# RobotControlLab/nimblephysics

Measured on AMD Instinct MI355X. Metric: differentiable timesteps/sec (fwd+bwd), 1024-env Atlas w/ contact, higher is better.
Workload: dtype f64; 1 GPU; Atlas 33-DoF (atlas_v3_box_colliders) + ground, foot contact; worlds_per_gpu=1024, dofs=33, global_batch=1024, parallelism=independent worlds x1, launcher=single process

## Files before the change

### nimblephysics_amd/csrc/capi.cpp

```cpp
#include <hip/hip_runtime.h>

#include <cmath>
#include <cstdlib>
#include <cstdio>
#include <cstring>
#include <string>
#include <vector>

#include "model.h"
#include "pool_sizes.h"

static thread_local std::string g_err;

static int fail(int code, const std::string& msg) {
  g_err = msg;
  return code;
}

#define HIP_TRY(expr)                                                        \
  do {                                                                       \
    hipError_t _e = (expr);                                                  \
    if (_e != hipSuccess) return fail(NIMBLE_ERR_HIP, std::string(#expr) + ": " + hipGetErrorString(_e)); \
  } while (0)

// ... 106 lines not shown
  m.ns = d->num_shapes;
  m.dt = d->dt;
  for (int i = 0; i < 3; i++) m.g[i] = d->gravity[i];
  m.clipDepth = d->contact_clipping_depth;
  m.fallbackCfm = d->fallback_cfm;
  m.penCorr = d->penetration_correction;
  m.parallelPosVel = d->parallel_pos_vel;
  int dofCount = 0;
  for (int b = 0; b < m.nb; b++) {
    int p = d->parent[b];
    if (p >= b) { delete w; return fail(NIMBLE_ERR_INVALID, "bodies must be in topological order"); }
    m.parent[b] = p;
    m.jtype[b] = d->joint_type[b];
    m.dof0[b] = d->dof_offset[b];
    m.ndof[b] = jointDofs(m.jtype[b]);
    if (m.ndof[b] < 0) { delete w; return fail(NIMBLE_ERR_INVALID, "unknown joint type"); }
    m.depth[b] = p >= 0 ? m.depth[p] + 1 : 0;
    if (m.depth[b] > m.maxDepth) m.maxDepth = m.depth[b];
    m.anc[b] = (p >= 0 ? m.anc[p] : 0ull) | (1ull << b);
    m.skel[b] = d->skeleton[b];
    std::memcpy(m.Tpj[b], d->T_parent_joint + 12 * b, 12 * sizeof(double));
    std::memcpy(m.Tcj[b], d->T_child_joint + 12 * b, 12 * sizeof(double));
    isoInverse(m.Tcj[b], m.TcjInv[b]);
    for (int i = 0; i < 3; i++) m.axis[b][i] = d->axis[3 * b + i];
    m.mass[b] = d->mass[b];
    for (int i = 0; i < 3; i++) m.com[b][i] = d->com[3 * b + i];
    const double* mo = d->moment + 6 * b;
    double I[9] = {mo[0], mo[3], mo[4], mo[3], mo[1], mo[5], mo[4], mo[5], mo[2]};
    std::memcpy(m.Ic[b], I, sizeof(I));
    m.friction[b] = d->friction[b];
    m.restitution[b] = d->restitution[b];
    for (int k = 0; k < m.ndof[b]; k++) m.dofBody[m.dof0[b] + k] = b;
    dofCount += m.ndof[b];
    if (m.jtype[b] == NIMBLE_JOINT_FREE || m.jtype[b] == NIMBLE_JOINT_BALL) {
      if (m.numFree >= 8) { delete w; return fail(NIMBLE_ERR_UNSUPPORTED, "more than 8 free / ball joints"); }
      m.freeBody[m.numFree++] = b;
    }
  }
  if (dofCount != m.n) { delete w; return fail(NIMBLE_ERR_INVALID, "dof count mismatch"); }
  {
    int k = 0;
    for (int lev = 0; lev <= m.maxDepth; lev++) {
      m.levelStart[lev] = k;
      for (int b = 0; b < m.nb; b++)
        if (m.depth[b] == lev) m.levelBodies[k++] = b;
    }
    m.levelStart[m.maxDepth + 1] = k;
    k = 0;
    for (int p = 0; p < m.nb; p++) {
      m.childStart[p] = k;
      for (int b = 0; b < m.nb; b++)
        if (m.parent[b] == p) m.childList[k++] = b;
    }
    m.childStart[m.nb] = k;
    k = 0;
    for (int lev = m.maxDepth; lev >= 1; lev--)
      for (int b = 0; b < m.nb; b++)
        if (m.depth[b] == lev && m.parent[b] >= 0) { m.accEdge[k][0] = m.parent[b]; m.accEdge[k][1] = b; k++; }
    m.numAcc = k;
  }
  for (int b = 0; b < m.nb; b++) {
    bool hasDof = false;
    for (int a = b; a >= 0; a = m.parent[a]) if (m.ndof[a] > 0) { hasDof = true; break; }
    m.reactive[b] = (d->skeleton_mobile[b] && hasDof) ? 1 : 0;
  }
  for (int i = 0; i < m.n; i++) {
    m.damping[i] = d->damping[i]; m.spring[i] = d->spring[i]; m.rest[i] = d->rest_position[i];
    m.posLo[i] = d->pos_lower[i]; m.posHi[i] = d->pos_upper[i];
    m.velLo[i] = d->vel_lower[i]; m.velHi[i] = d->vel_upper[i];
    m.forceLo[i] = d->force_lower[i]; m.forceHi[i] = d->force_upper[i];
  }
  for (int sIdx = 0; sIdx < m.ns; sIdx++) {
    m.shapeBody[sIdx] = d->shape_body[sIdx];
    m.shapeType[sIdx] = d->shape_type[sIdx];
    for (int i = 0; i < 3; i++) m.shapeSize[sIdx][i] = d->shape_size[3 * sIdx + i];
    std::memcpy(m.shapeT[sIdx], d->shape_T + 12 * sIdx, 12 * sizeof(double));
  }
  m.helperPrio = 0;
  if (const char* e = getenv("NIMBLE_AMD_HELPER_PRIO")) m.helperPrio = atoi(e) & 3;
  m.postSplit = 1;
  if (const char* e = getenv("NIMBLE_AMD_POST_SPLIT")) m.postSplit = atoi(e) != 0;
  m.pinvMfma = 1;
  if (const char* e = getenv("NIMBLE_AMD_PINV_MFMA")) m.pinvMfma = atoi(e) != 0 ? 1 : 0;
  m.guardSites = 0;
  m.guardStride = 1;
  m.guardOffset = 0;
  if (const char* e = getenv("NIMBLE_AMD_GUARD_TEST")) {
    int sites = 0, stride = 1, offset = 0;
    if (sscanf(e, "%d:%d:%d", &sites, &stride, &offset) >= 1 && stride > 0 && offset >= 0 && offset < stride) {
      m.guardSites = sites;
      m.guardStride = stride;
      m.guardOffset = offset;
    }
  }
  m.numPairs = 0;
  m.pairChunk = 0;
  for (int i = 0; i < m.ns; i++)
    for (int j = i + 1; j < m.ns; j++) {
      int bi = m.shapeBody[i], bj = m.shapeBody[j];
      if (bi == bj) continue;
      int si = m.skel[bi], sj = m.skel[bj];
      if (!d->skeleton_mobile[bi] && !d->skeleton_mobile[bj]) continue;
      if (si == sj) continue;
      m.pairA[m.numPairs] = i;
      m.pairB[m.numPairs] = j;
      m.numPairs++;
    }
  m.pairChunk = m.numPairs < CT_PAIR_CHUNK_HOST ? m.numPairs : CT_PAIR_CHUNK_HOST;
  {
    std::vector<double> mv;
    m.hasMesh = 0;
    for (int sIdx = 0; sIdx < m.ns; sIdx++) {
      m.meshFirst[sIdx] = 0; m.meshCount[sIdx] = 0; m.meshRadius[sIdx] = 0.0;
      if (m.shapeType[sIdx] != NIMBLE_SHAPE_MESH) continue;
      if (d->mesh_vertices == nullptr || d->shape_mesh_count == nullptr || d->shape_mesh_count[sIdx] <= 0) {
        delete w;
        return fail(NIMBLE_ERR_INVALID, "mesh shape without vertices");
      }
      const int f = d->shape_mesh_first[sIdx], c = d->shape_mesh_count[sIdx];
      if (f < 0 || f + c > d->num_mesh_vertices) { delete w; return fail(NIMBLE_ERR_INVALID, "mesh vertex range"); }
      m.meshFirst[sIdx] = (int)(mv.size() / 3);
      double r2 = 0.0;
      for (int k = 0; k < c; k++) {
        const double* v = d->mesh_vertices + 3 * (size_t)(f + k);
        double q = 0.0;
        for (int i = 0; i < 3; i++) q += (v[i] * m.shapeSize[sIdx][i]) * (v[i] * m.shapeSize[sIdx][i]);
        if (q > r2) r2 = q;
        if (d->mesh_vertex_candidate != nullptr && d->mesh_vertex_candidate[f + k] == 0) continue;
        mv.insert(mv.end(), v, v + 3);
      }
      m.meshCount[sIdx] = (int)(mv.size() / 3) - m.meshFirst[sIdx];
      m.meshRadius[sIdx] = std::sqrt(r2);
      if (m.meshCount[sIdx] <= 0) {
        delete w;
        return fail(NIMBLE_ERR_INVALID, "mesh_vertex_candidate filters out every vertex of a mesh shape");
      }
    }
    if (!mv.empty()) {
      hipError_t e = hipMalloc(&w->meshDev, mv.size() * sizeof(double));
      if (e == hipSuccess) e = hipMemcpy(w->meshDev, mv.data(), mv.size() * sizeof(double), hipMemcpyHostToDevice);
      if (e != hipSuccess) {
        if (w->meshDev) (void)hipFree(w->meshDev);
        delete w;
        return fail(NIMBLE_ERR_HIP, std::string("mesh upload: ") + hipGetErrorString(e));
      }
    }
    m.meshVerts = w->meshDev;
    for (int p = 0; p < m.numPairs; p++)
      if (m.shapeType[m.pairA[p]] == NIMBLE_SHAPE_MESH || m.shapeType[m.pairB[p]] == NIMBLE_SHAPE_MESH) m.hasMesh = 1;
    if (m.hasMesh) m.pairChunk = m.numPairs > 0 ? 1 : 0;
  }
  int maxContacts = m.hasMesh ? NIMBLE_MAX_CONTACTS : 8 * m.numPairs;
  if (maxContacts > NIMBLE_MAX_CONTACTS) maxContacts = NIMBLE_MAX_CONTACTS;
  m.maxContacts = maxContacts;
  const int mcap = 3 * maxContacts < NIMBLE_MAX_SOLVED_LCP ? 3 * maxContacts : NIMBLE_MAX_SOLVED_LCP;
  if (const char* e = getenv("NIMBLE_AMD_DEFER_ROWS")) {
    const int d = atoi(e);
    if (d >= 0 && d < w->deferRows) w->deferRows = d;
  }
  int fwdRows = ldsPoolRows(m, mcap);
  for (;;) {
    w->fwd = makeLayout(m, false, fwdRows);
    if (w->fwd.total * 8 <= 160 * 1024) break;
    if (fwdRows == 0) {
      if (w->meshDev) (void)hipFree(w->meshDev);
      delete w;
// ... 251 lines not shown
```

### nimblephysics_amd/csrc/contact.cuh

```cuda
#pragma once
#include "model.h"
#include "spatial.cuh"
#include "pool_sizes.h"
#include "capsule.cuh"
#include "mesh.cuh"

#define CT_FACE_VERTEX 1
#define CT_VERTEX_FACE 2
#define CT_EDGE_EDGE 3
#include "stamp.cuh"

#define CM_CLAMPING (-1)
#define CM_NOT_CLAMPING (-2)


__device__ int deviceBoxBox(const double* p1, const double* R1, const double* A, const double* p2,
                            const double* R2, const double* B, double clipDepth, int b1, int b2, double* out) {
#pragma clang fp contract(off)
  const double fudge = 1.05;
  double p[3] = {p2[0] - p1[0], p2[1] - p1[1], p2[2] - p1[2]};
  double pp[3];
  for (int i = 0; i < 3; i++) pp[i] = R1[i] * p[0] + R1[3 + i] * p[1] + R1[6 + i] * p[2];
  double Rm[9], Qm[9];
  for (int i = 0; i < 3; i++)
// ... 2612 lines not shown
    }
  }
  const double tn = sqrt(dot3(t, t));
  for (int i = 0; i < 3; i++) t[i] /= tn;
  double gc[3];
  cross3(cr, g, gc);
  for (int i = 0; i < 3; i++) gc[i] /= tn;
  double gt[3];
  if (fabs(tn - 1.0) > 1e-6) {
    const double dd = dot3(gc, t);
    for (int i = 0; i < 3; i++) gt[i] = gc[i] - dd * t[i];
  } else {
    for (int i = 0; i < 3; i++) gt[i] = gc[i];
  }
  double a[3], b[3];
  cross3(g, t, a);
  cross3(nrm, gt, b);
  for (int i = 0; i < 3; i++) { T0[i] = gt[i]; T1[i] = a[i] + b[i]; }
}

template <int R = 1>
__device__ int contactBackwardPrep(const ModelDev& md, double* s, const Layout& L, int lane, const double* sn,
                                   BwdPool& P, int m, int nc, double* ct, int fcRow) {
  const int n = md.n;
  const double dt = md.dt;
  const double* rows = sn + SN_ROWS;
  const double* Ac = sn + snAc(n);
  const double* AcubE = sn + snAcubE(n);
  const double* PT = sn + snPT(n);
  const double* Q = sn + snQ(n);
  const double* Lm = s + L.M;
  const double* dinv = s + L.dinv;
  const int imp = uni((int)sn[SN_IMP]);
#ifdef NIMBLE_STAGE_TIMING
  double* g_stamp = (double*)sn + snStamps(n);
#endif
  STAMP(30);
  (void)ct;
  for (int j = lane; j < m; j += WAVE)
    if ((int)rows[j * SN_ROWREC + RR_MAP] == CM_CLAMPING) P.rowOf[(int)rows[j * SN_ROWREC + RR_CIDX]] = j;
  WSYNC();
  for (int c = lane; c < nc; c += WAVE) {
    const int r = P.rowOf[c];
    P.fc[c] = sn[SN_FC + c];
    P.bc[c] = rows[r * SN_ROWREC + RR_B];
    P.bounce[c] = rows[r * SN_ROWREC + RR_BOUNCE];
  }
  WSYNC();
  for (int c = lane; c < nc; c += WAVE) {
    double xx = 0;
#pragma unroll 8
    for (int r = 0; r < nc; r++) xx += PT[r * nc + c] * P.bc[r];
    P.xq[c] = xx;
  }
  WSYNC();
  for (int c = lane; c < nc; c += WAVE) {
    double qx = 0, ze = 0;
    if (imp)
#pragma unroll 8
      for (int k = 0; k < nc; k++) {
        qx += Q[c * nc + k] * P.xq[k];
        ze += PT[c * nc + k] * P.xq[k];
      }
    P.r1[c] = imp ? P.bc[c] - qx : 0.0;
    P.zeta[c] = imp ? ze : 0.0;
  }
  WSYNC();
  STAMP(31);
  {
    double X[5] = {0, 0, 0, 0, 0};
    if (lane < n) {
      X[0] = s[L.gv + lane];
      double a1 = 0, a2 = 0, a3 = 0, a4 = 0;
#pragma unroll 8
      for (int c = 0; c < nc; c++) {
        const double ae = AcubE[lane * nc + c], ac = Ac[lane * nc + c];
        a1 += ae * P.fc[c];
        a2 += ae * P.xq[c];
        a3 += ac * P.r1[c];
        a4 += ac * P.zeta[c];
      }
      X[1] = a1; X[2] = a2; X[3] = a3; X[4] = a4;
    }
    cholSolveReg<5>(Lm, dinv, X, n, lane);
    if (lane < n) {
      double* nv = P.NV + lane * NV_COLS;
      const double d = X[1] / dt;
      nv[NV_W] = X[0];
      nv[NV_DELTA] = d;
      nv[NV_SIGMA] = X[2];
      nv[NV_MA1] = X[3];
      nv[NV_MA2] = X[4];
      s[L.w + lane] = X[0];
      s[L.x + lane] = sn[snYf(n) + lane] + d;
    }
  }
  WSYNC();
  for (int c = lane; c < nc; c += WAVE) {
    double acc = 0;
#pragma unroll 8
    for (int i = 0; i < n; i++) acc += AcubE[i * nc + c] * s[L.w + i];
    P.u[c] = fcRow >= 0 ? (c == fcRow ? 1.0 : 0.0) : acc;
  }
  WSYNC();
  for (int c = lane; c < nc; c += WAVE) {
    double l = 0;
#pragma unroll 8
    for (int r = 0; r < nc; r++) l += PT[c * nc + r] * P.u[r];
    P.lam[c] = l;
    P.beta[c] = P.bounce[c] * l;
  }
  WSYNC();
  for (int c = lane; c < nc; c += WAVE) {
    double qtl = 0, rh = 0;
    if (imp)
#pragma unroll 8
      for (int k = 0; k < nc; k++) {
        qtl += Q[k * nc + c] * P.lam[k];
        rh += PT[k * nc + c] * P.lam[k];
      }
    P.piv[c] = imp ? P.u[c] - qtl : 0.0;
    P.rho[c] = imp ? rh : 0.0;
  }
  WSYNC();
  STAMP(35);
  {
    double X[4] = {0, 0, 0, 0};
    double mu = 0;
    if (lane < n) {
      double a0 = 0, a1 = 0, a2 = 0, a3 = 0;
#pragma unroll 8
      for (int c = 0; c < nc; c++) {
        const double ae = AcubE[lane * nc + c], ac = Ac[lane * nc + c];
        a0 += ac * P.beta[c];
        a1 += ac * P.lam[c];
        a2 += ae * P.rho[c];
        a3 += ae * P.piv[c];
      }
      X[0] = a0; X[1] = a1; X[2] = a2; X[3] = a3;
      mu = a0;
    }
    cholSolveReg<4>(Lm, dinv, X, n, lane);
    if (lane < n) {
      double* nv = P.NV + lane * NV_COLS;
      nv[NV_MU] = mu;
      nv[NV_NU] = X[0];
      nv[NV_KAPPA] = X[1];
      nv[NV_MARHO] = X[2];
      nv[NV_MAPI] = X[3];
      const double w2 = nv[NV_W] - X[0];
      nv[NV_W2] = w2;
      s[L.w + lane] = w2;
    }
  }
  WSYNC();
  STAMP(37);
  int rMap[R], rC[R];
  double rE[R];
#pragma unroll
  for (int q = 0; q < R; q++) {
    const int j = rowAt(q, lane);
    rMap[q] = CM_NOT_CLAMPING;
    rC[q] = 0;
    rE[q] = 0.0;
    if (j < m) {
      const double* rr = rows + j * SN_ROWREC;
      rMap[q] = (int)rr[RR_MAP];
      if (rMap[q] == CM_CLAMPING) rC[q] = (int)rr[RR_CIDX];
      else if (rMap[q] >= 0) { rC[q] = (int)rows[rMap[q] * SN_ROWREC + RR_CIDX]; rE[q] = rr[RR_EVAL]; }
    }
  }
  {
    const int i = lane;
    const bool live = i < n;
    const double* nv = P.NV + (live ? i : 0) * NV_COLS;
    const double w = nv[NV_W], sg = nv[NV_SIGMA], ka = nv[NV_KAPPA], ma1 = nv[NV_MA1], mar = nv[NV_MARHO];
    const double ma2 = nv[NV_MA2], map = nv[NV_MAPI], vf = sn[SN_VF + (live ? i : 0)];
    for (int j = 0; j < m; j++) {
      const int mp = rdliR(rMap, j);
      const int c = rdliR(rC, j);
      const double e = rdlR(rE, j);
      double g = 0.0;
      if (mp == CM_CLAMPING) {
        g = P.fc[c] * w - P.beta[c] * vf - P.lam[c] * sg - P.xq[c] * ka;
        if (imp) g += P.rho[c] * ma1 + P.r1[c] * mar + P.piv[c] * ma2 + P.zeta[c] * map;
      } else if (mp >= 0) {
        double inner = P.fc[c] * w - P.xq[c] * ka;
        if (imp) inner += P.rho[c] * ma1 + P.piv[c] * ma2;
        g = e * inner;
      }
      if (live) P.gRows[j * n + i] = g;
    }
  }
  WSYNC();
  {
    auto bodyOf = [&](int t) {
      if (t >= 2 * m) return -1;
      const double* rec = sn + SN_CONTACTS + (int)rows[(t >> 1) * SN_ROWREC + RR_CONTACT] * CREC;
      return (int)rec[8 + (t & 1)];
    };
    unsigned long long anAll = 0ull;
    for (int t = lane; t < 2 * m; t += WAVE) {
      const int body = bodyOf(t);
      if (body >= 0) anAll |= md.anc[body];
    }
    unsigned lo = (unsigned)anAll, hi = (unsigned)(anAll >> 32);
    for (int o = 32; o >= 1; o >>= 1) {
      lo |= __shfl_xor(lo, o);
      hi |= __shfl_xor(hi, o);
    }
    const unsigned long long all = ((unsigned long long)uni((int)hi) << 32) | (unsigned)uni((int)lo);
    const unsigned long long dmAll = ancestorDofMask(md, all, lane);
    for (int t0 = 0; t0 < 2 * m; t0 += WAVE) {
      const int t = t0 + lane;
      const int body = bodyOf(t);
      const unsigned long long an = body >= 0 ? md.anc[body] : 0ull;
      unsigned long long dm = dmAll;
      double T[6] = {0, 0, 0, 0, 0, 0};
      const double* g = P.gRows + (t < 2 * m ? (t >> 1) : 0) * n;
      while (dm) {
        const int r = __ffsll((long long)dm) - 1;
        dm &= dm - 1ull;
        const double gr = ((an >> md.dofBody[r]) & 1ull) ? g[r] : 0.0;
        for (int i = 0; i < 6; i++) T[i] = fma(s[L.Sw + 6 * r + i], gr, T[i]);
// ... 511 lines not shown
      {
        unsigned long long dm = ancestorDofMask(md, md.anc[c], lane);
        if (lane < nb) {
          double pb[6] = {0, 0, 0, 0, 0, 0};
          const unsigned long long an = md.anc[lane];
          while (dm) {
            const int r = __ffsll((long long)dm) - 1;
            dm &= dm - 1ull;
            const double w = ((an >> md.dofBody[r]) & 1ull) ? 1.0 : 0.0;
#pragma unroll
            for (int i = 0; i < 6; i++) pb[i] = fma(w, omega[6 * r + i], pb[i]);
          }
          for (int i = 0; i < 6; i++) Pc[lane * 6 + i] = pb[i];
        }
      }
      WSYNC();
      if (k < n && ((md.anc[c] >> bk) & 1ull)) {
        double y[6];
        for (int i = 0; i < 6; i++) y[i] = Pc[c * 6 + i] - (lam >= 0 ? Pc[lam * 6 + i] : 0.0);
        acc += dot6(Z, y);
        const double zw = sqrt(Z[0] * Z[0] + Z[1] * Z[1] + Z[2] * Z[2]);
        if (zw > 1e-6) acc += Z[0] * UV[3] + Z[1] * UV[4] + Z[2] * UV[5];
        acc += Z[3] * UV[0] + Z[4] * UV[1] + Z[5] * UV[2];
      }
      WSYNC();
      TACC_END(83, tP);
      if (lane == 0 && g_stamp) g_stamp[85] += 1;
    }
  }
  TACC_BEGIN(tF);
  {
#pragma unroll
    for (int q = 0; q < R; q++)
    for (unsigned long long bits = liveRows[q]; bits; bits &= bits - 1ull) {
      const int j = 64 * q + __ffsll((long long)bits) - 1;
      const int A = rdliR(rA, j), B = rdliR(rB, j), type = rdliR(rTyp, j) & 15;
      const int con = rdliR(rCon, j), dirIdx = rdliR(rDir, j);
      double p[3], nrm[3];
      for (int i = 0; i < 3; i++) { p[i] = rdlR(rp[i], j); nrm[i] = rdlR(rn[i], j); }
      if (k >= n) continue;
      if (type >= CT_EDGE_EDGE) {
        const double* rr = rows + j * SN_ROWREC;
        const double* rec = sn + SN_CONTACTS + con * CREC;
        if (type == CT_EDGE_EDGE) acc += edgeRowTerm(md, P, j, rec, rr, sn + snEdge(n) + con * EDGE_REC, Z, bk, A, B);
        else if (type == CT_SPHERE_SPHERE)
          acc += sphereSphereRowTerm(md, P, j, rec, rr, sn + snEdge(n) + con * EDGE_REC, Z, bk, A, B);
        else if (type == CT_PIPE_PIPE)
          acc += pipePipeRowTerm(md, P, j, rec, rr, sn + snEdge(n) + con * EDGE_REC, Z, bk, A, B);
        else if (type == CT_SPHERE_PIPE || type == CT_PIPE_SPHERE)
          acc += spherePipeRowTerm(md, P, j, rec, rr, sn + snEdge(n) + con * EDGE_REC, Z, bk, A, B, type);
        else if (type >= CT_PIPE_VERTEX && type <= CT_EDGE_PIPE)
          acc += pipeMeshRowTerm(md, P, j, rec, rr, sn + snEdge(n) + con * EDGE_REC, Z, bk, A, B, type);
        else acc += sphereRowTerm(md, s, L, P, j, rec, rr, Z, bk);
        continue;
      }
      int faceBody = -1;
      if (type == CT_VERTEX_FACE) faceBody = B;
      else if (type == CT_FACE_VERTEX) faceBody = A;
      if (faceBody < 0 || !((md.anc[faceBody] >> bk) & 1ull)) continue;
      double dn[3];
      const double wv[3] = {Z[0], Z[1], Z[2]};
      cross3(wv, nrm, dn);
      double dd[3];
      if (dirIdx == 0 || dot3(dn, dn) <= 1e-12) {
        for (int i = 0; i < 3; i++) dd[i] = dn[i];
      } else {
        double T0[3], T1[3];
        tangentBasisGradient(nrm, dn, T0, T1);
        for (int i = 0; i < 3; i++) dd[i] = dirIdx == 1 ? T0[i] : T1[i];
      }
      double pxdd[3];
      cross3(p, dd, pxdd);
      double v = 0.0;
      for (int i = 0; i < 3; i++)
        v += (P.TAB[j * 12 + i] - P.TAB[j * 12 + 6 + i]) * pxdd[i] +
             (P.TAB[j * 12 + 3 + i] - P.TAB[j * 12 + 9 + i]) * dd[i];
      acc += v;
    }
  }
  TACC_END(84, tF);
  return acc;
}

__device__ double mFieldsTerm(const ModelDev& md, double* s, const Layout& L, const double* NV, double* buf, int lane,
                              int k, const double* Z, double coefDelta, double imp) {
  const int nb = md.nb;
  const double coef[4] = {coefDelta, 1.0, -imp, -imp};
  double* wI = buf + 24 * nb;
  if (lane < nb) {
    const int b = lane;
    const double* Tw = s + L.Tw + 12 * b;
    const double m = md.mass[b];
    double cw[3], Rc[9], tmp[9];
    for (int r = 0; r < 3; r++)
      cw[r] = Tw[r * 4] * md.com[b][0] + Tw[r * 4 + 1] * md.com[b][1] + Tw[r * 4 + 2] * md.com[b][2] + Tw[r * 4 + 3];
    for (int r = 0; r < 3; r++)
      for (int c = 0; c < 3; c++)
        tmp[r * 3 + c] = Tw[r * 4] * md.Ic[b][c] + Tw[r * 4 + 1] * md.Ic[b][3 + c] + Tw[r * 4 + 2] * md.Ic[b][6 + c];
    for (int r = 0; r < 3; r++)
      for (int c = 0; c < 3; c++)
        Rc[r * 3 + c] = tmp[r * 3] * Tw[c * 4] + tmp[r * 3 + 1] * Tw[c * 4 + 1] + tmp[r * 3 + 2] * Tw[c * 4 + 2];
    const double C[9] = {0, -cw[2], cw[1], cw[2], 0, -cw[0], -cw[1], cw[0], 0};
    double* w = wI + 13 * b;
    for (int r = 0; r < 3; r++)
      for (int c = 0; c < 3; c++) {
        const double cct = C[r * 3] * C[c * 3] + C[r * 3 + 1] * C[c * 3 + 1] + C[r * 3 + 2] * C[c * 3 + 2];
        w[r * 3 + c] = Rc[r * 3 + c] + m * cct;
      }
    w[9] = cw[0]; w[10] = cw[1]; w[11] = cw[2]; w[12] = m;
  }
  WSYNC();
  double total = 0.0;
  const int npairs = imp != 0.0 ? 4 : 2;
  for (int pr = 0; pr < npairs; pr++) {
    if (lane < nb) {
      const int b = lane;
      double Va[6] = {0, 0, 0, 0, 0, 0}, Vc[6] = {0, 0, 0, 0, 0, 0};
      const unsigned long long an = md.anc[b];
      const double* ga = NV + 2 * pr;
      const double* gc = NV + 2 * pr + 1;
#pragma unroll 4
      for (int r = 0; r < md.n; r++) {
        const bool in = (an >> md.dofBody[r]) & 1ull;
        const double xa = in ? ga[r * NV_COLS] : 0.0, xc = in ? gc[r * NV_COLS] : 0.0;
        const double* S = s + L.Sw + 6 * r;
        for (int i = 0; i < 6; i++) {
          Va[i] = fma(S[i], xa, Va[i]);
          Vc[i] = fma(S[i], xc, Vc[i]);
        }
      }
      const double* w = wI + 13 * b;
      const double m = w[12];
      const double C[9] = {0, -w[11], w[10], w[11], 0, -w[9], -w[10], w[9], 0};
      double I[36];
      for (int r = 0; r < 3; r++)
        for (int c = 0; c < 3; c++) {
          I[r * 6 + c] = w[r * 3 + c];
          I[r * 6 + c + 3] = m * C[r * 3 + c];
          I[(r + 3) * 6 + c] = m * C[c * 3 + r];
          I[(r + 3) * 6 + c + 3] = (r == c) ? m : 0.0;
        }
      double* Fa = buf + b * 12;
      double* Fc = buf + (nb + b) * 12;
      double ha[6], hc[6];
      mv6(I, Va, ha);
      mv6(I, Vc, hc);
      for (int i = 0; i < 6; i++) { Fa[i] = Va[i]; Fa[6 + i] = ha[i]; Fc[i] = Vc[i]; Fc[6 + i] = hc[i]; }
    }
    WSYNC();
    if (lane < 12) {
      double* base = buf + (lane < 6 ? 0 : nb * 12) + 6 + (lane % 6);
#pragma unroll 4
      for (int k = 0; k < md.numAcc; k++) {
        const int p = md.accEdge[k][0], c = md.accEdge[k][1];
        base[p * 12] += base[c * 12];
      }
    }
    WSYNC();
    const int bk = k < md.n ? md.dofBody[k] : 0;
    double ha[6], hc[6];
    for (int i = 0; i < 6; i++) { ha[i] = buf[bk * 12 + 6 + i]; hc[i] = buf[(nb + bk) * 12 + 6 + i]; }
    if (k < md.n) {
      const int lam = md.parent[bk];
      double val = 0.0;
      if (lam >= 0) {
        double t[6];
        crm(Z, buf + (nb + lam) * 12, t);
        val -= dot6(t, ha);
        crm(Z, buf + lam * 12, t);
        val -= dot6(t, hc);
      }
      total += coef[pr] * val;
    }
    WSYNC();
  }
  return total;
}
```

### nimblephysics_amd/csrc/model.h

```cpp
#pragma once
#include <stdint.h>

#include "../../include/nimble_amd.h"

inline int jointDofs(int jt) {
  switch (jt) {
    case NIMBLE_JOINT_WELD: return 0;
    case NIMBLE_JOINT_REVOLUTE: case NIMBLE_JOINT_PRISMATIC: return 1;
    case NIMBLE_JOINT_BALL: case NIMBLE_JOINT_TRANSLATIONAL: return 3;
    case NIMBLE_JOINT_FREE: return 6;
    default: return -1;
  }
}

#define NB_MAX NIMBLE_MAX_BODIES
#define ND_MAX NIMBLE_MAX_DOFS
#define NS_MAX NIMBLE_MAX_SHAPES

struct Layout {
  int q, v, tau, Tw, Sw, V, A, IC, F, M, rhs, x, scratch;
  int adj, Wt, w, gp, gv;
  int ct, v1, pool, poolCap, dinv;
  int snDyn;
  int cscr;
  int stage, stageCap;
  int early;
  int total;
};

struct ModelDev {
  int nb, n, ns, maxDepth;
  int numFree;
  int freeBody[8];
  double dt, g[3], clipDepth, fallbackCfm;
  int penCorr, parallelPosVel;
  int parent[NB_MAX], jtype[NB_MAX], dof0[NB_MAX], ndof[NB_MAX], depth[NB_MAX];
  int skel[NB_MAX], reactive[NB_MAX];
  unsigned long long anc[NB_MAX];
  int levelStart[NB_MAX + 1], levelBodies[NB_MAX];
  int childStart[NB_MAX + 1], childList[NB_MAX];
  int numAcc;
  int accEdge[NB_MAX][2];
  double Tpj[NB_MAX][12];
  double Tcj[NB_MAX][12];
  double TcjInv[NB_MAX][12];
  double axis[NB_MAX][3];
  double mass[NB_MAX], com[NB_MAX][3], Ic[NB_MAX][9];
  double friction[NB_MAX], restitution[NB_MAX];
  int dofBody[ND_MAX];
  double damping[ND_MAX], spring[ND_MAX], rest[ND_MAX];
  double posLo[ND_MAX], posHi[ND_MAX], velLo[ND_MAX], velHi[ND_MAX], forceLo[ND_MAX], forceHi[ND_MAX];
  int shapeBody[NS_MAX], shapeType[NS_MAX];
  double shapeSize[NS_MAX][3];
  double shapeT[NS_MAX][12];
  const double* meshVerts;
  int meshFirst[NS_MAX], meshCount[NS_MAX];
  double meshRadius[NS_MAX];
  int hasMesh;
  int helperPrio;
  int postSplit;
  int pinvMfma;
  int guardSites, guardStride, guardOffset;
  int maxContacts;
  int numPairs, pairChunk;
  int pairA[NS_MAX * (NS_MAX - 1) / 2], pairB[NS_MAX * (NS_MAX - 1) / 2];
  Layout lay[2];
};
```

### nimblephysics_amd/csrc/timestep.hip

```cpp
#include <hip/hip_runtime.h>

#include "model.h"
#include "spatial.cuh"
#include "wave.cuh"
#include "stamp.cuh"
#include "chol_wave.cuh"

#define WAVE 64

__device__ __forceinline__ void ancestorAccelerations(const ModelDev& md, double* s, const Layout& L, int lane,
                                                      const double* ddq, double* X);
__device__ __forceinline__ void kinematics(const ModelDev& md, double* s, const Layout& L, int lane, const double* ddq,
                                           double* g_stamp = nullptr) {
  (void)g_stamp;
  STAMP(70);
  const double* q = s + L.q;
  const double* v = s + L.v;
  if (lane < md.nb) {
    const int b = lane;
    const int jt = md.jtype[b];
    const int o = md.dof0[b];
    double Q[12] = {1, 0, 0, 0, 0, 1, 0, 0, 0, 0, 1, 0};
    const double* a = md.axis[b];
    if (jt == NIMBLE_JOINT_REVOLUTE) {
// ... 512 lines not shown

__device__ void rightJacobianCol(const double* th, int k, double* o) {
  const double t2 = th[0] * th[0] + th[1] * th[1] + th[2] * th[2];
  const double t = sqrt(t2);
  double a, b;
  if (t < 1e-3) { a = 0.5; b = 1.0 / 6.0; }
  else { a = (1.0 - cos(t)) / t2; b = (t - sin(t)) / (t2 * t); }
  const double K[9] = {0, -th[2], th[1], th[2], 0, -th[0], -th[1], th[0], 0};
  for (int r = 0; r < 3; r++) {
    double k2 = K[r * 3] * K[k] + K[r * 3 + 1] * K[3 + k] + K[r * 3 + 2] * K[6 + k];
    o[r] = (r == k ? 1.0 : 0.0) - a * K[r * 3 + k] + b * k2;
  }
}

template <int R>
__device__ __forceinline__ void backwardItems(const ModelDev* __restrict__ mdp, int batch,
                                              const double* __restrict__ state, const double* __restrict__ forces,
                                              double* __restrict__ snapshot, int snapDoubles,
                                              const double* __restrict__ gradNext, double* __restrict__ gradState,
                                              double* __restrict__ gradForces, int rows, double* __restrict__ ws,
                                              int wsDoubles, double* __restrict__ gradMasses, int fcMode,
                                              int massParams, int deferRows) {
  extern __shared__ double s[];
  const ModelDev& md = *mdp;
  const Layout& L = md.lay[1];
  const int lane = threadIdx.x;
  const int n = md.n;
  const double dt = md.dt;
  const long long items = (long long)batch * rows;
  for (long long item = blockIdx.x; item < items; item += gridDim.x) {
    const int env = rows == 1 ? (int)item : (int)(item / rows);
    const int unitRow = rows == 1 ? -1 : (int)(item - (long long)env * rows);
    if (md.numPairs > 0) {
      const int mEnv = uni((int)snapshot[(size_t)env * snapDoubles + SN_M]);
      if ((mEnv > deferRows) != (R > 1)) continue;
    }
#ifdef NIMBLE_STAGE_TIMING
    double* g_stamp = md.numPairs > 0 ? snapshot + (size_t)env * snapDoubles + snStamps(n) : nullptr;
#endif
    STAMP(20);
    if (fcMode && (md.numPairs == 0 || unitRow >= uni((int)snapshot[(size_t)env * snapDoubles + SN_NC]))) {
      for (int i = lane; i < 2 * n; i += WAVE) gradState[(size_t)item * 2 * n + i] = 0.0;
      for (int i = lane; i < n; i += WAVE) gradForces[(size_t)item * n + i] = 0.0;
      continue;
    }
    loadState(md, s, L, lane, state + (size_t)env * 2 * n, forces + (size_t)env * n);
    if (fcMode) {
      for (int i = lane; i < n; i += WAVE) { s[L.gp + i] = 0.0; s[L.gv + i] = 0.0; }
    } else if (unitRow < 0) {
      const double* gN = gradNext + (size_t)env * 2 * n;
      for (int i = lane; i < n; i += WAVE) {
        s[L.gp + i] = gN[i];
        s[L.gv + i] = gN[n + i];
      }
    } else {
      for (int i = lane; i < n; i += WAVE) {
        s[L.gp + i] = i == unitRow ? 1.0 : 0.0;
        s[L.gv + i] = n + i == unitRow ? 1.0 : 0.0;
      }
    }
    double* sn = snapshot + (size_t)env * snapDoubles;
    double* hbmWs = ws != nullptr ? ws + (size_t)blockIdx.x * wsDoubles : sn + snapWorkspaceOffset(n);
    dynCacheCopy(md, s, L, sn + L.snDyn, false, lane);
    STAMP(21);
    const int nc = md.numPairs > 0 ? uni((int)sn[SN_NC]) : 0;
    const int m = md.numPairs > 0 ? uni((int)sn[SN_M]) : 0;
    double* x = s + L.x;
    double* w = s + L.w;
    BwdPool P;
    int imp = 0;
    if (nc > 0) {
      const int need = bwdPoolDoubles(m, n);
      carveBwd(need <= L.poolCap ? s + L.pool : hbmWs, m, n, P);
      imp = contactBackwardPrep<R>(md, s, L, lane, sn, P, m, nc, s + L.ct, fcMode ? unitRow : -1);
    } else {
      for (int i = lane; i < n; i += WAVE) {
        const double qi = s[L.q + i], vi = s[L.v + i];
        const double springF = md.spring[i] * (qi - md.rest[i] + dt * vi);
        const double dampF = md.damping[i] * vi;
        x[i] = dt * (s[L.tau + i] - s[L.rhs + i] - dampF - springF);
        w[i] = s[L.gv + i];
      }
      WSYNC();
      cholSolve(s + L.M, s + L.dinv, x, n, lane);
      cholSolve(s + L.M, s + L.dinv, w, n, lane);
      for (int i = lane; i < n; i += WAVE) x[i] /= dt;
      WSYNC();
    }
    STAMP(22);
    accelerations(md, s, L, lane, x, s + L.adj);
    adjointVectors(md, s, L, lane);
    STAMP(23);

    double gq = 0.0, gvOut = 0.0, gt = 0.0;
    double Z[6] = {0, 0, 0, 0, 0, 0};
    const int k = lane;
    if (k < n) {
      const int b = md.dofBody[k];
      const int lam = md.parent[b];
      const double ag[6] = {0, 0, 0, md.g[0], md.g[1], md.g[2]};
      double Vl[6], ul[6];
      for (int i = 0; i < 6; i++) {
        Vl[i] = lam >= 0 ? s[L.V + 6 * lam + i] : 0.0;
        ul[i] = (lam >= 0 ? s[L.A + 6 * lam + i] : 0.0) - ag[i];
      }
      const double* Sk = s + L.Sw + 6 * k;
      if (md.jtype[b] == NIMBLE_JOINT_FREE || md.jtype[b] == NIMBLE_JOINT_BALL) {
        const int o = md.dof0[b];
        const int c = k - o;
        double xi[6] = {0, 0, 0, 0, 0, 0};
        const double* th = s + L.q + o;
        if (c < 3) {
          rightJacobianCol(th, c, xi);
        } else {
          double Rm[9];
          expMapRot(th, Rm);
          for (int r = 0; r < 3; r++) xi[3 + r] = Rm[(c - 3) * 3 + r];
        }
        double TwC[12];
        tmul(s + L.Tw + 12 * b, md.Tcj[b], TwC);
        adT(TwC, xi, Z);
      } else {
        for (int i = 0; i < 6; i++) Z[i] = Sk[i];
      }
      const double* a = s + L.adj + 42 * b;
      double t[6], r[6], acc6[6];
      crf(Vl, a + 6, t);
      for (int i = 0; i < 6; i++) r[i] = a[12 + i] + t[i] + a[24 + i] - a[30 + i];
      crf(Vl, r, t);
      crf(ul, a + 6, r);
      for (int i = 0; i < 6; i++) acc6[i] = -a[i] - r[i] + t[i] + a[18 + i] + a[36 + i];
      const double accQ = dot6(Z, acc6);
      double vs[6];
      for (int i = 0; i < 6; i++) vs[i] = Vl[i] + s[L.V + 6 * b + i];
      crf(vs, a + 6, t);
      for (int i = 0; i < 6; i++) acc6[i] = -t[i] - a[12 + i] - a[24 + i] + a[30 + i];
      const double accV = dot6(Sk, acc6);
      const double wk = w[k];
      gq = -dt * accQ - dt * md.spring[k] * wk;
      gvOut = s[L.gv + k] - dt * accV - dt * md.damping[k] * wk - dt * dt * md.spring[k] * wk;
      gt = dt * wk;
      if (nc > 0) gvOut -= P.NV[k * NV_COLS + NV_MU];
      if (md.jtype[b] != NIMBLE_JOINT_FREE && md.jtype[b] != NIMBLE_JOINT_BALL) {
        gq += s[L.gp + k];
        gvOut += dt * s[L.gp + k];
      }
    }
    WSYNC();
    STAMP(24);
    if (nc > 0) {
      double* buf = s + L.adj;
      TACC_BEGIN(tG);
#ifdef NIMBLE_STAGE_TIMING
      const double gterm = contactGTermsAll<R>(md, s, L, sn, P, m, Z, buf, lane, g_stamp);
#else
      const double gterm = contactGTermsAll<R>(md, s, L, sn, P, m, Z, buf, lane);
#endif
      WSYNC();
      TACC_END(80, tG);
      TACC_BEGIN(tM);
      const double mterm = mFieldsTerm(md, s, L, P.NV, buf, lane, k, Z, -dt, (double)imp);
      TACC_END(81, tM);
      if (k < n) {
        gq += gterm;
        gq += mterm;
      }
      WSYNC();
    }
    STAMP(25);
    if (gradMasses != nullptr) {
      if (lane < md.nb) {
        const int b = lane;
        const double* Tw = s + L.Tw + 12 * b;
        const double m = md.mass[b];
        double cw[3];
        for (int r = 0; r < 3; r++)
          cw[r] = Tw[r * 4] * md.com[b][0] + Tw[r * 4 + 1] * md.com[b][1] + Tw[r * 4 + 2] * md.com[b][2] + Tw[r * 4 + 3];
        auto comVel = [&](const double* y, double* u) {
          double cx[3];
          cross3(cw, y, cx);
          for (int i = 0; i < 3; i++) u[i] = y[3 + i] - cx[i];
        };
        auto bodyAng = [&](const double* y, double* wb) {
          for (int i = 0; i < 3; i++) wb[i] = Tw[i] * y[0] + Tw[4 + i] * y[1] + Tw[8 + i] * y[2];
        };
        auto pairTerms = [&](const double* x, const double* y, double coef, double* out) {
          double ux[3], uy[3];
          comVel(x, ux);
          comVel(y, uy);
          out[0] += coef * (ux[0] * uy[0] + ux[1] * uy[1] + ux[2] * uy[2]);
          if (massParams < 10) return;
          for (int k = 0; k < 3; k++) {
            const double rk[3] = {Tw[k], Tw[4 + k], Tw[8 + k]};
            double a[3], c[3];
            cross3(x, rk, a);
            cross3(y, rk, c);
            out[1 + k] += coef * m * (a[0] * uy[0] + a[1] * uy[1] + a[2] * uy[2] + ux[0] * c[0] + ux[1] * c[1] + ux[2] * c[2]);
          }
          double bx[3], by[3];
          bodyAng(x, bx);
          bodyAng(y, by);
          out[4] += coef * bx[0] * by[0];
          out[5] += coef * bx[1] * by[1];
          out[6] += coef * bx[2] * by[2];
          out[7] += coef * (bx[0] * by[1] + bx[1] * by[0]);
          out[8] += coef * (bx[0] * by[2] + bx[2] * by[0]);
          out[9] += coef * (bx[1] * by[2] + bx[2] * by[1]);
        };
        const double ag[6] = {0, 0, 0, md.g[0], md.g[1], md.g[2]};
        const double* Vb = s + L.V + 6 * b;
        double Ab[6], Vw[6], val[10] = {0, 0, 0, 0, 0, 0, 0, 0, 0, 0};
        for (int i = 0; i < 6; i++) Ab[i] = s[L.A + 6 * b + i] - ag[i];
        bodyTwist(md, s + L.Sw, b, s + L.w, 1, Vw);
        pairTerms(Vw, Ab, -dt, val);
        {
          double uV[3], h[6], fh[6];
          comVel(Vb, uV);
          cross3(cw, uV, h);
          for (int i = 0; i < 3; i++) h[3 + i] = uV[i];
          crf(Vb, h, fh);
          val[0] += -dt * dot6(Vw, fh);
          if (massParams >= 10) {
            double bv[3];
            bodyAng(Vb, bv);
            for (int k = 0; k < 3; k++) {
              const double rk[3] = {Tw[k], Tw[4 + k], Tw[8 + k]};
              double du[3], t1[3], t2[3];
              cross3(Vb, rk, du);
              cross3(rk, uV, t1);
              cross3(cw, du, t2);
              for (int i = 0; i < 3; i++) { h[i] = m * (t1[i] + t2[i]); h[3 + i] = m * du[i]; }
              crf(Vb, h, fh);
              val[1 + k] += -dt * dot6(Vw, fh);
            }
            const int pi[6] = {0, 1, 2, 0, 0, 1}, pj[6] = {0, 1, 2, 1, 2, 2};
            for (int q = 0; q < 6; q++) {
              double eb[3] = {0, 0, 0};
              eb[pi[q]] += bv[pj[q]];
              if (pi[q] != pj[q]) eb[pj[q]] += bv[pi[q]];
              for (int i = 0; i < 3; i++) { h[i] = Tw[i * 4] * eb[0] + Tw[i * 4 + 1] * eb[1] + Tw[i * 4 + 2] * eb[2]; h[3 + i] = 0.0; }
              crf(Vb, h, fh);
              val[4 + q] += -dt * dot6(Vw, fh);
            }
          }
// ... 61 lines not shown
```

Baseline: 3.102 million timesteps/s.

## Fuse backward M-field passes pairwise and batch the two no-contact Cholesky solves

After: 3.154 million timesteps/s, median of 6. 1.7% higher.

```diff
diff --git a/nimblephysics_amd/csrc/capi.cpp b/nimblephysics_amd/csrc/capi.cpp
--- a/nimblephysics_amd/csrc/capi.cpp
+++ b/nimblephysics_amd/csrc/capi.cpp
@@ -212,6 +212,10 @@
   if (const char* e = getenv("NIMBLE_AMD_POST_SPLIT")) m.postSplit = atoi(e) != 0;
   m.pinvMfma = 1;
   if (const char* e = getenv("NIMBLE_AMD_PINV_MFMA")) m.pinvMfma = atoi(e) != 0 ? 1 : 0;
+  m.bwdMFuse = 1;
+  if (const char* e = getenv("NIMBLE_AMD_BWD_MFUSE")) m.bwdMFuse = atoi(e) != 0 ? 1 : 0;
+  m.bwdSolve2 = 1;
+  if (const char* e = getenv("NIMBLE_AMD_BWD_SOLVE2")) m.bwdSolve2 = atoi(e) != 0 ? 1 : 0;
   m.guardSites = 0;
   m.guardStride = 1;
   m.guardOffset = 0;
diff --git a/nimblephysics_amd/csrc/contact.cuh b/nimblephysics_amd/csrc/contact.cuh
--- a/nimblephysics_amd/csrc/contact.cuh
+++ b/nimblephysics_amd/csrc/contact.cuh
@@ -2718,7 +2718,9 @@
       }
       X[1] = a1; X[2] = a2; X[3] = a3; X[4] = a4;
     }
+    STAMP(32);
     cholSolveReg<5>(Lm, dinv, X, n, lane);
+    STAMP(33);
     if (lane < n) {
       double* nv = P.NV + lane * NV_COLS;
       const double d = X[1] / dt;
@@ -2776,6 +2778,7 @@
       X[0] = a0; X[1] = a1; X[2] = a2; X[3] = a3;
       mu = a0;
     }
+    STAMP(36);
     cholSolveReg<4>(Lm, dinv, X, n, lane);
     if (lane < n) {
       double* nv = P.NV + lane * NV_COLS;
@@ -3453,11 +3456,103 @@
   return acc;
 }
 
-__device__ double mFieldsTerm(const ModelDev& md, double* s, const Layout& L, const double* NV, double* buf, int lane,
-                              int k, const double* Z, double coefDelta, double imp) {
+template <int NP>
+__device__ __forceinline__ double mFieldPasses(const ModelDev& md, const double* s, const Layout& L, const double* NV,
+                                               int ldNV, double* buf, const double* wI, int lane, int k, const double* Z,
+                                               const double (&coef)[4], int npairs
+#ifdef NIMBLE_STAGE_TIMING
+                                               , double* g_stamp
+#endif
+) {
+  constexpr int NF = 2 * NP;
+  const int nb = md.nb;
+  double total = 0.0;
+  for (int p0 = 0; p0 < npairs; p0 += NP) {
+    TACC_BEGIN(tV);
+    if (lane < nb) {
+      const int b = lane;
+      double V[NF][6];
+      for (int f = 0; f < NF; f++)
+        for (int i = 0; i < 6; i++) V[f][i] = 0.0;
+      const unsigned long long an = md.anc[b];
+      const double* g = NV + 2 * p0;
+#pragma unroll 4
+      for (int r = 0; r < md.n; r++) {
+        const bool in = (an >> md.dofBody[r]) & 1ull;
+        double xf[NF];
+        for (int f = 0; f < NF; f++) xf[f] = in ? g[r * ldNV + f] : 0.0;
+        const double* S = s + L.Sw + 6 * r;
+        for (int i = 0; i < 6; i++)
+          for (int f = 0; f < NF; f++) V[f][i] = fma(S[i], xf[f], V[f][i]);
+      }
+      const double* w = wI + 13 * b;
+      const double m = w[12];
+      const double C[9] = {0, -w[11], w[10], w[11], 0, -w[9], -w[10], w[9], 0};
+      double I[36];
+      for (int r = 0; r < 3; r++)
+        for (int c = 0; c < 3; c++) {
+          I[r * 6 + c] = w[r * 3 + c];
+          I[r * 6 + c + 3] = m * C[r * 3 + c];
+          I[(r + 3) * 6 + c] = m * C[c * 3 + r];
+          I[(r + 3) * 6 + c + 3] = (r == c) ? m : 0.0;
+        }
+      for (int f = 0; f < NF; f++) {
+        double* F = buf + (f * nb + b) * 12;
+        double h[6];
+        mv6(I, V[f], h);
+        for (int i = 0; i < 6; i++) { F[i] = V[f][i]; F[6 + i] = h[i]; }
+      }
+    }
+    WSYNC();
+    TACC_END(52, tV);
+    TACC_BEGIN(tW);
+    if (lane < 6 * NF) {
+      double* base = buf + (lane / 6) * nb * 12 + 6 + (lane % 6);
+#pragma unroll 4
+      for (int e = 0; e < md.numAcc; e++) {
+        const int p = md.accEdge[e][0], c = md.accEdge[e][1];
+        base[p * 12] += base[c * 12];
+      }
+    }
+    WSYNC();
+    TACC_END(53, tW);
+    TACC_BEGIN(tR);
+    const int bk = k < md.n ? md.dofBody[k] : 0;
+    for (int q = 0; q < NP; q++) {
+      const double* Fa = buf + 2 * q * nb * 12;
+      const double* Fc = buf + (2 * q + 1) * nb * 12;
+      double ha[6], hc[6];
+      for (int i = 0; i < 6; i++) { ha[i] = Fa[bk * 12 + 6 + i]; hc[i] = Fc[bk * 12 + 6 + i]; }
+      if (k < md.n) {
+        const int lam = md.parent[bk];
+        double val = 0.0;
+        if (lam >= 0) {
+          double t[6];
+          crm(Z, Fc + lam * 12, t);
+          val -= dot6(t, ha);
+          crm(Z, Fa + lam * 12, t);
+          val -= dot6(t, hc);
+        }
+        total += coef[p0 + q] * val;
+      }
+    }
+    WSYNC();
+    TACC_END(59, tR);
+#ifdef NIMBLE_STAGE_TIMING
+    if (lane == 0 && g_stamp) g_stamp[89] += 1.0;
+#endif
+  }
+  return total;
+}
+
+__device__ double mFieldsTerm(const ModelDev& md, double* s, const Layout& L, const double* NV, int ldNV, double* buf,
+                              double* wI, bool fuse, int lane, int k, const double* Z, double coefDelta, double imp
+#ifdef NIMBLE_STAGE_TIMING
+                              , double* g_stamp
+#endif
+) {
   const int nb = md.nb;
   const double coef[4] = {coefDelta, 1.0, -imp, -imp};
-  double* wI = buf + 24 * nb;
   if (lane < nb) {
     const int b = lane;
     const double* Tw = s + L.Tw + 12 * b;
@@ -3481,69 +3576,12 @@
     w[9] = cw[0]; w[10] = cw[1]; w[11] = cw[2]; w[12] = m;
   }
   WSYNC();
-  double total = 0.0;
   const int npairs = imp != 0.0 ? 4 : 2;
-  for (int pr = 0; pr < npairs; pr++) {
-    if (lane < nb) {
-      const int b = lane;
-      double Va[6] = {0, 0, 0, 0, 0, 0}, Vc[6] = {0, 0, 0, 0, 0, 0};
-      const unsigned long long an = md.anc[b];
-      const double* ga = NV + 2 * pr;
-      const double* gc = NV + 2 * pr + 1;
-#pragma unroll 4
-      for (int r = 0; r < md.n; r++) {
-        const bool in = (an >> md.dofBody[r]) & 1ull;
-        const double xa = in ? ga[r * NV_COLS] : 0.0, xc = in ? gc[r * NV_COLS] : 0.0;
-        const double* S = s + L.Sw + 6 * r;
-        for (int i = 0; i < 6; i++) {
-          Va[i] = fma(S[i], xa, Va[i]);
-          Vc[i] = fma(S[i], xc, Vc[i]);
-        }
-      }
-      const double* w = wI + 13 * b;
-      const double m = w[12];
-      const double C[9] = {0, -w[11], w[10], w[11], 0, -w[9], -w[10], w[9], 0};
-      double I[36];
-      for (int r = 0; r < 3; r++)
-        for (int c = 0; c < 3; c++) {
-          I[r * 6 + c] = w[r * 3 + c];
-          I[r * 6 + c + 3] = m * C[r * 3 + c];
-          I[(r + 3) * 6 + c] = m * C[c * 3 + r];
-          I[(r + 3) * 6 + c + 3] = (r == c) ? m : 0.0;
-        }
-      double* Fa = buf + b * 12;
-      double* Fc = buf + (nb + b) * 12;
-      double ha[6], hc[6];
-      mv6(I, Va, ha);
-      mv6(I, Vc, hc);
-      for (int i = 0; i < 6; i++) { Fa[i] = Va[i]; Fa[6 + i] = ha[i]; Fc[i] = Vc[i]; Fc[6 + i] = hc[i]; }
-    }
-    WSYNC();
-    if (lane < 12) {
-      double* base = buf + (lane < 6 ? 0 : nb * 12) + 6 + (lane % 6);
-#pragma unroll 4
-      for (int k = 0; k < md.numAcc; k++) {
-        const int p = md.accEdge[k][0], c = md.accEdge[k][1];
-        base[p * 12] += base[c * 12];
-      }
-    }
-    WSYNC();
-    const int bk = k < md.n ? md.dofBody[k] : 0;
-    double ha[6], hc[6];
-    for (int i = 0; i < 6; i++) { ha[i] = buf[bk * 12 + 6 + i]; hc[i] = buf[(nb + bk) * 12 + 6 + i]; }
-    if (k < md.n) {
-      const int lam = md.parent[bk];
-      double val = 0.0;
-      if (lam >= 0) {
-        double t[6];
-        crm(Z, buf + (nb + lam) * 12, t);
-        val -= dot6(t, ha);
-        crm(Z, buf + lam * 12, t);
-        val -= dot6(t, hc);
-      }
-      total += coef[pr] * val;
-    }
-    WSYNC();
-  }
-  return total;
-}
+#ifdef NIMBLE_STAGE_TIMING
+  if (fuse) return mFieldPasses<2>(md, s, L, NV, ldNV, buf, wI, lane, k, Z, coef, npairs, g_stamp);
+  return mFieldPasses<1>(md, s, L, NV, ldNV, buf, wI, lane, k, Z, coef, npairs, g_stamp);
+#else
+  if (fuse) return mFieldPasses<2>(md, s, L, NV, ldNV, buf, wI, lane, k, Z, coef, npairs);
+  return mFieldPasses<1>(md, s, L, NV, ldNV, buf, wI, lane, k, Z, coef, npairs);
+#endif
+}
diff --git a/nimblephysics_amd/csrc/model.h b/nimblephysics_amd/csrc/model.h
--- a/nimblephysics_amd/csrc/model.h
+++ b/nimblephysics_amd/csrc/model.h
@@ -60,6 +60,8 @@
   int helperPrio;
   int postSplit;
   int pinvMfma;
+  int bwdMFuse;
+  int bwdSolve2;
   int guardSites, guardStride, guardOffset;
   int maxContacts;
   int numPairs, pairChunk;
diff --git a/nimblephysics_amd/csrc/timestep.hip b/nimblephysics_amd/csrc/timestep.hip
--- a/nimblephysics_amd/csrc/timestep.hip
+++ b/nimblephysics_amd/csrc/timestep.hip
@@ -618,8 +618,16 @@
         w[i] = s[L.gv + i];
       }
       WSYNC();
-      cholSolve(s + L.M, s + L.dinv, x, n, lane);
-      cholSolve(s + L.M, s + L.dinv, w, n, lane);
+      if (md.bwdSolve2) {
+        double xw[2] = {lane < n ? x[lane] : 0.0, lane < n ? w[lane] : 0.0};
+        cholSolveReg<2>(s + L.M, s + L.dinv, xw, n, lane);
+        WSYNC();
+        if (lane < n) { x[lane] = xw[0]; w[lane] = xw[1]; }
+        WSYNC();
+      } else {
+        cholSolve(s + L.M, s + L.dinv, x, n, lane);
+        cholSolve(s + L.M, s + L.dinv, w, n, lane);
+      }
       for (int i = lane; i < n; i += WAVE) x[i] /= dt;
       WSYNC();
     }
@@ -695,7 +703,33 @@
       WSYNC();
       TACC_END(80, tG);
       TACC_BEGIN(tM);
-      const double mterm = mFieldsTerm(md, s, L, P.NV, buf, lane, k, Z, -dt, (double)imp);
+      bool mfuse = false;
+      double* wI = buf + 24 * md.nb;
+      const double* NVf = P.NV;
+      int ldNV = NV_COLS;
+      if (md.bwdMFuse) {
+        const int wId = (13 * md.nb + 1) & ~1;
+        const bool onChip = bwdPoolDoubles(m, n) <= L.poolCap;
+        int idle = onChip ? 0 : L.poolCap;
+        double* free = s + L.pool;
+        if (n * (n + 1) / 2 >= wId) { mfuse = true; wI = s + L.M; }
+        else if (onChip && (n + 12) * m >= wId) { mfuse = true; wI = P.gRows; }
+        else if (idle >= wId) { mfuse = true; wI = free; free += wId; idle -= wId; }
+        if (mfuse) {
+          if (idle >= 8 * n) {
+            double* stage = free;
+            if (lane < n)
+              for (int c = 0; c < 8; c++) stage[lane * 8 + c] = P.NV[lane * NV_COLS + c];
+            NVf = stage;
+            ldNV = 8;
+          }
+        }
+      }
+#ifdef NIMBLE_STAGE_TIMING
+      const double mterm = mFieldsTerm(md, s, L, NVf, ldNV, buf, wI, mfuse, lane, k, Z, -dt, (double)imp, g_stamp);
+#else
+      const double mterm = mFieldsTerm(md, s, L, NVf, ldNV, buf, wI, mfuse, lane, k, Z, -dt, (double)imp);
+#endif
       TACC_END(81, tM);
       if (k < n) {
         gq += gterm;
```
